# databendlabs/databend

Measured on AMD Instinct MI355X. Metric: rows/s TPC-H Q1 hash-agg, higher is better.
Workload: dtype i64/i128 decimal

## Files before the change

### databend_amd/csrc/k_parquet_dev.hip

```cpp
#include "pq_common.h"

#include <stdlib.h>
#include "dv_wave.h"

namespace {

enum { DV_OK = 0, DV_CORRUPT = 1, DV_UNSUPPORTED = 2 };
enum { ENC_DELTA_BINARY_PACKED = 5, ENC_DELTA_LENGTH_BYTE_ARRAY = 6, ENC_DELTA_BYTE_ARRAY = 7, ENC_BYTE_STREAM_SPLIT = 9 };
__host__ __device__ __forceinline__ bool dv_ext_enc(uint32_t e) {
  return e == ENC_DELTA_LENGTH_BYTE_ARRAY || e == ENC_DELTA_BYTE_ARRAY || e == ENC_BYTE_STREAM_SPLIT;
}
enum { CODEC_NONE = 0, CODEC_SNAPPY = 1, CODEC_ZSTD = 6, CODEC_LZ4_RAW = 7 };
enum { PQ_NODE_LIST = 1, PQ_NODE_STRUCT = 2 };
inline uint32_t bit_width_u32(uint32_t v) { uint32_t b = 0; for (; v; v >>= 1) ++b; return b; }

__device__ __forceinline__ void dv_fail(uint32_t* ctl, uint32_t code) { atomicCAS(&ctl[0], 0u, code); }

__device__ __forceinline__ uint32_t uni(uint32_t v) { return (uint32_t)__builtin_amdgcn_readfirstlane((int)v); }

__global__ __launch_bounds__(128) void dv_inflate_zstd2_kernel(const DvJob* __restrict__ jobs, uint32_t ring) {
  extern __shared__ __align__(16) uint8_t dv_lds[];
  const DvJob P = jobs[blockIdx.x];
  const uint32_t lane = threadIdx.x & 63, wave = threadIdx.x >> 6;
  const uint32_t lev = P.lev_len;
  const uint32_t raw = P.compressed ? lev : P.uncomp_len;
  for (uint32_t i = threadIdx.x; i < raw; i += 128) P.dst[i] = P.src[i];
  if (!P.compressed || P.uncomp_len == lev) return;
  ZQueue Q;
  Q.slots = (u32x4q*)(dv_lds + ring + ZW_TABLES);
  Q.ctl = (uint32_t*)(dv_lds + ring + ZW_TABLES + ZQ_CAP * 16);
  if (threadIdx.x < 4) Q.ctl[threadIdx.x] = 0;
  __syncthreads();
  if (wave == 0) {
    ZProd a;
    a.begin(P, dv_lds, ring, lane);
    a.qbegin(Q);
    int rc = zc::decode_frames(a, a.in_len);
    if (rc == zc::OK && a.op_ != a.cap_) rc = zc::CORRUPT_;
    a.end((uint32_t)rc);
  } else {
    ZWave b;
    b.begin(P, dv_lds, ring, lane);
    const int rc = (int)zq_consume(b, Q);
    b.flush(true);
    if (rc) dv_fail(P.ctl, rc == zc::UNSUPPORTED ? DV_UNSUPPORTED : DV_CORRUPT);
  }
}

__global__ __launch_bounds__(64) void dv_inflate_lz_kernel(const DvJob* __restrict__ jobs, uint32_t ring) {
  extern __shared__ __align__(16) uint8_t dv_lds[];
  const DvJob P = jobs[blockIdx.x];
  const uint32_t lane = threadIdx.x;
  const uint32_t lev = P.lev_len;
  const uint32_t raw = P.compressed ? lev : P.uncomp_len;
  for (uint32_t i = lane; i < raw; i += 64) P.dst[i] = P.src[i];
  if (!P.compressed || P.uncomp_len == lev) return;
  ZWave w;
  w.begin(P, dv_lds, ring, lane);
  FwdStream in;
  in.open(w.srcA, w.safeA, w.a0, lane);
  bool ok = P.codec == CODEC_SNAPPY ? snappy_raw(w, in) : lz4_block(w, in);
  if (ok && w.op_ != w.cap_) ok = false;
  w.flush(true);
  if (!ok) dv_fail(P.ctl, DV_CORRUPT);
}

__device__ __forceinline__ uint64_t dv_peek8(const uint8_t* __restrict__ s, uint32_t pos, uint32_t len) {
  uint64_t v = 0;
#pragma unroll
  for (int k = 0; k < 8; ++k)
    if (pos + (uint32_t)k < len) v |= (uint64_t)s[pos + k] << (8 * k);
  return v;
}

__device__ __forceinline__ bool dv_varint(const uint8_t* __restrict__ s, uint32_t* pos, uint32_t len, uint64_t* out) {
  const uint64_t w = dv_peek8(s, *pos, len);
  uint64_t v = 0;
  for (int k = 0; k < 8; ++k) {
    if (*pos + (uint32_t)k >= len) return false;
    const uint32_t b = (uint32_t)(w >> (8 * k)) & 0xFFu;
    v |= (uint64_t)(b & 0x7F) << (7 * k);
    if (!(b & 0x80)) { *pos += (uint32_t)k + 1; *out = v; return true; }
  }
  for (int k = 8; k < 10; ++k) {
    if (*pos + (uint32_t)k >= len) return false;
    const uint32_t b = s[*pos + k];
    v |= (uint64_t)(b & 0x7F) << (7 * k);
    if (!(b & 0x80)) { *pos += (uint32_t)k + 1; *out = v; return true; }
  }
  return false;
}

template <class Rle, class Bp>
__device__ __forceinline__ bool dv_walk_hybrid(const uint8_t* __restrict__ s, uint32_t len, int bitw, uint32_t nvals, Rle&& rle, Bp&& bp) {
// ... 490 lines not shown
  } else if (cv.esize == 16) {
    ((i128*)out)[o] = (i128)(int64_t)v;
  } else {
    ((uint64_t*)out)[o] = v;
  }
}

__device__ __forceinline__ uint64_t dv_unpack64(const uint8_t* __restrict__ src, uint32_t i, uint32_t b) {
  if (b == 0) return 0;
  const uint64_t bit = (uint64_t)i * b;
  const uint8_t* p = src + (bit >> 3);
  const uint32_t sh = (uint32_t)(bit & 7);
  const uint32_t nb = (sh + b + 7) >> 3;
  uint64_t v = load_le(p, nb < 8 ? (int)nb : 8) >> sh;
  if (nb > 8) v |= (uint64_t)p[8] << (64 - sh);
  return b >= 64 ? v : (v & ((1ull << b) - 1));
}

struct DvDeltaShared {
  uint64_t wt[4];
};

template <class Put>
__device__ __forceinline__ bool dv_delta_walk(const uint8_t* __restrict__ s, uint32_t rlen, uint32_t count, bool exact, DvDeltaShared* S, Put&& put,
                                              uint32_t* end) {
  const uint32_t tid = threadIdx.x;
  uint32_t pos = 0;
  uint64_t bs, mb, total, zz;
  if (!dv_varint(s, &pos, rlen, &bs) || !dv_varint(s, &pos, rlen, &mb) || !dv_varint(s, &pos, rlen, &total) || !dv_varint(s, &pos, rlen, &zz))
    return false;
  if (mb == 0 || mb > 4096 || bs == 0 || bs > (1u << 24) || bs % mb != 0) return false;
  const uint32_t vpm = (uint32_t)(bs / mb);
  if (vpm % 8 != 0) return false;
  if (total < (uint64_t)count || (exact && total != (uint64_t)count)) return false;
  *end = pos;
  if (count == 0) return true;
  uint64_t last = (zz >> 1) ^ (0 - (zz & 1));
  if (tid == 0) put(0u, last);
  uint32_t produced = 1;
  while (produced < count) {
    uint64_t mz;
    if (!dv_varint(s, &pos, rlen, &mz)) return false;
    const uint64_t min_delta = (mz >> 1) ^ (0 - (mz & 1));
    if (rlen - pos < (uint32_t)mb) return false;
    const uint32_t bwpos = pos;
    pos += (uint32_t)mb;
    for (uint32_t m = 0; m < (uint32_t)mb && produced < count; ++m) {
      const uint32_t b = s[bwpos + m];
      if (b > 64) return false;
      const uint32_t need = (count - produced) < vpm ? (count - produced) : vpm;
      const uint64_t need_bytes = ((uint64_t)need * b + 7) >> 3;
      if ((uint64_t)(rlen - pos) < need_bytes) return false;
      for (uint32_t c0 = 0; c0 < need; c0 += 256) {
        const uint32_t i = c0 + tid;
        const uint64_t dlt = i < need ? min_delta + dv_unpack64(s + pos, i, b) : 0;
        uint64_t incl = dlt;
        for (int dd = 1; dd < 64; dd <<= 1) {
          const uint64_t t = __shfl_up(incl, dd, 64);
          if ((int)(tid & 63) >= dd) incl += t;
        }
        __syncthreads();
        if ((tid & 63) == 63) S->wt[tid >> 6] = incl;
        __syncthreads();
        uint64_t wb = last;
        for (uint32_t w = 0; w < (tid >> 6); ++w) wb += S->wt[w];
        if (i < need) put(produced + i, wb + incl);
        last += S->wt[0] + S->wt[1] + S->wt[2] + S->wt[3];
      }
      const uint64_t mbytes = ((uint64_t)vpm * b) >> 3;
      pos += mbytes < (uint64_t)(rlen - pos) ? (uint32_t)mbytes : rlen - pos;
      produced += need;
    }
  }
  *end = pos;
  return true;
}

__device__ bool dv_delta(const uint8_t* __restrict__ s, uint32_t rlen, uint32_t count, const PqConv& cv, void* __restrict__ out, uint64_t o0,
                         DvDeltaShared* S) {
  uint32_t end;
  return dv_delta_walk(s, rlen, count, false, S, [&](uint32_t i, uint64_t v) { dv_store_int(cv, out, o0 + i, v); }, &end);
}

__device__ __forceinline__ void dv_put_dict(const PqConv& cv, const void* __restrict__ dict, uint32_t idx, void* __restrict__ out, uint64_t o) {
  switch (cv.esize) {
    case 1: ((uint8_t*)out)[o] = ((const uint8_t*)dict)[idx]; break;
    case 2: ((uint16_t*)out)[o] = ((const uint16_t*)dict)[idx]; break;
    case 4: ((uint32_t*)out)[o] = ((const uint32_t*)dict)[idx]; break;
    case 8: ((uint64_t*)out)[o] = ((const uint64_t*)dict)[idx]; break;
    default: ((uint4*)out)[o] = ((const uint4*)dict)[idx]; break;
  }
}

union DvValShared {
  DvStrShared str;
  DvDeltaShared delta;
};

__global__ __launch_bounds__(256) void dv_dict_kernel(const DvChunkD* __restrict__ cds, const uint32_t* __restrict__ list) {
  __shared__ DvStrShared S;
  const DvChunkD& C = cds[list[blockIdx.x]];
  const uint8_t* __restrict__ img = C.img;
  const PqConv cv = C.cv;
  void* __restrict__ dict = C.dict_out;
  uint32_t* __restrict__ ctl = C.hdr;
  const DvPage P = C.pages[C.dict_page];
  if (P.num_values == 0) return;
  if (cv.physical == PT_BYTE_ARRAY) {
    if (!dv_walk_strings(img, P.img_off, P.uncomp_len, P.num_values, dict, 0, &S)) dv_fail(ctl, DV_CORRUPT);
    return;
  }
  const uint32_t w = (uint32_t)plain_width(cv.physical, cv.type_length);
  if (w == 0 || P.uncomp_len / w < P.num_values) { dv_fail(ctl, DV_CORRUPT); return; }
  for (uint32_t i = threadIdx.x; i < P.num_values; i += 256) store_plain(cv, img + P.img_off + (uint64_t)i * w, dict, i);
}

__global__ __launch_bounds__(256) void dv_values_kernel(const DvChunkD* __restrict__ cds, const uint2* __restrict__ map) {
  __shared__ DvValShared S;
  const uint2 m = map[blockIdx.x];
  const DvChunkD& C = cds[m.x];
  if (blockIdx.y >= C.slices) return;
  const uint32_t d = m.y, tid = threadIdx.x;
  const uint8_t* __restrict__ img = C.img;
  const PqConv cv = C.cv;
  const void* __restrict__ dict = C.dict;
  const uint32_t dict_n = C.dict_n;
  void* __restrict__ out = C.target;
  const uint64_t out_cap = C.rows;
  uint32_t* __restrict__ ctl = C.hdr;
  const DvPage P = C.pages[C.dp[d]];
  const uint32_t n = C.nn[d], vo = C.voff[d];
  const uint64_t o0 = C.vbase[d];
  if (n == 0) return;
  if (vo > P.uncomp_len || n > P.num_values || o0 + n > out_cap) { dv_fail(ctl, DV_CORRUPT); return; }
  const uint8_t* s = img + P.img_off + vo;
  const uint32_t rlen = P.uncomp_len - vo;
  const uint32_t enc = P.enc;
  if (enc == ENC_PLAIN && cv.physical != PT_BOOLEAN && cv.physical != PT_BYTE_ARRAY) {
    const uint32_t w = (uint32_t)plain_width(cv.physical, cv.type_length);
    if (w == 0 || rlen / w < n) { dv_fail(ctl, DV_CORRUPT); return; }
    const uint32_t lo = (uint32_t)((uint64_t)n * blockIdx.y / C.slices), hi = (uint32_t)((uint64_t)n * (blockIdx.y + 1) / C.slices);
    for (uint32_t i = lo + tid; i < hi; i += 256) store_plain(cv, s + (uint64_t)i * w, out, o0 + i);
    return;
  }
  if (blockIdx.y != 0) return;
  bool ok = true;
  if (enc == ENC_PLAIN && cv.physical == PT_BOOLEAN) {
    if ((uint64_t)rlen * 8 < n) { dv_fail(ctl, DV_CORRUPT); return; }
    (void)dv_put_bits((uint32_t*)out, o0, n, s, tid, 256);
  } else if (enc == ENC_PLAIN) {
    ok = dv_walk_strings(img, P.img_off + vo, rlen, n, out, o0, &S.str);
  } else if (enc == ENC_PLAIN_DICT || enc == ENC_RLE_DICT) {
    if (rlen < 1 || dict_n == 0 || !dict) { dv_fail(ctl, DV_CORRUPT); return; }
    const int bitw = s[0];
    if (bitw > 32) { dv_fail(ctl, DV_CORRUPT); return; }
    ok = dv_walk_hybrid(
        s + 1, rlen - 1, bitw, n,
        [&](uint32_t first, uint32_t cnt, uint32_t v) {
          if (v >= dict_n) dv_fail(ctl, DV_CORRUPT);
          const uint32_t idx = v < dict_n ? v : dict_n - 1;
          for (uint32_t i = tid; i < cnt; i += 256) dv_put_dict(cv, dict, idx, out, o0 + first + i);
        },
        [&](uint32_t first, uint32_t cnt, const uint8_t* src) {
          for (uint32_t i = tid; i < cnt; i += 256) {
            uint32_t idx = extract_bits(src, i, bitw);
            if (idx >= dict_n) { dv_fail(ctl, DV_CORRUPT); idx = dict_n - 1; }
            dv_put_dict(cv, dict, idx, out, o0 + first + i);
          }
        });
  } else if (enc == ENC_RLE && cv.physical == PT_BOOLEAN) {
    if (rlen < 4) { dv_fail(ctl, DV_CORRUPT); return; }
    const uint32_t len = (uint32_t)load_le(s, 4);
    if (len > rlen - 4) { dv_fail(ctl, DV_CORRUPT); return; }
    ok = dv_walk_hybrid(
        s + 4, len, 1, n,
        [&](uint32_t first, uint32_t cnt, uint32_t v) { if (v == 1) (void)dv_put_bits((uint32_t*)out, o0 + first, cnt, nullptr, tid, 256); },
        [&](uint32_t first, uint32_t cnt, const uint8_t* src) { (void)dv_put_bits((uint32_t*)out, o0 + first, cnt, src, tid, 256); });
  } else if (enc == ENC_DELTA_BINARY_PACKED && (cv.physical == PT_INT32 || cv.physical == PT_INT64)) {
    ok = dv_delta(s, rlen, n, cv, out, o0, &S.delta);
  } else {
    dv_fail(ctl, DV_UNSUPPORTED);
    return;
  }
  if (!ok) dv_fail(ctl, DV_CORRUPT);
}

struct DvXJob {
  uint32_t k, d;
  uint32_t enc, sec;
  uint32_t* lens;
  uint8_t* dst;
  uint64_t aoff;
  uint64_t bytes;
  uint32_t live, pad;
};

__device__ __forceinline__ void dv_view(const uint8_t* __restrict__ p, uint32_t len, uint32_t buf, uint32_t off, void* __restrict__ out, uint64_t o) {
  uint32_t w[4];
  sv_make(p, len, buf, off, w);
  ((uint4*)out)[o] = make_uint4(w[0], w[1], w[2], w[3]);
}

__device__ __forceinline__ uint64_t dv_block_xscan(uint64_t v, uint64_t* wt, uint64_t* tot) {
  const uint32_t tid = threadIdx.x;
  uint64_t incl = v;
  for (int dd = 1; dd < 64; dd <<= 1) {
    const uint64_t t = __shfl_up(incl, dd, 64);
    if ((int)(tid & 63) >= dd) incl += t;
  }
  __syncthreads();
  if ((tid & 63) == 63) wt[tid >> 6] = incl;
  __syncthreads();
  uint64_t wb = 0;
  for (uint32_t w = 0; w < (tid >> 6); ++w) wb += wt[w];
  *tot = wt[0] + wt[1] + wt[2] + wt[3];
  return wb + incl - v;
}

__device__ __forceinline__ void dv_store_bss(const PqConv& cv, const uint8_t* __restrict__ s, uint32_t n, uint32_t i, void* __restrict__ out, uint64_t o) {
  if (cv.physical == PT_FLBA) {
    const int L = cv.type_length;
    u128 v = (s[i] & 0x80) ? ~(u128)0 : (u128)0;
#pragma unroll
    for (int b = 0; b < 16; ++b)
      if (b < L) v = (v << 8) | s[(uint64_t)b * n + i];
    if (cv.esize == 16) ((u128*)out)[o] = v; else ((uint64_t*)out)[o] = (uint64_t)v;
    return;
  }
  const int w = (cv.physical == PT_INT32 || cv.physical == PT_FLOAT) ? 4 : 8;
  uint64_t v = 0;
#pragma unroll
  for (int b = 0; b < 8; ++b)
    if (b < w) v |= (uint64_t)s[(uint64_t)b * n + i] << (8 * b);
  if (w == 4) {
    const uint32_t x = (uint32_t)v;
    switch (cv.esize) {
      case 1: ((uint8_t*)out)[o] = (uint8_t)x; break;
      case 2: ((uint16_t*)out)[o] = (uint16_t)x; break;
      case 4: ((uint32_t*)out)[o] = x; break;
      default: ((int64_t*)out)[o] = (int64_t)(int32_t)x; break;
    }
    return;
  }
  if (cv.esize == 16) ((i128*)out)[o] = (i128)(int64_t)v; else ((uint64_t*)out)[o] = v;
}

__global__ __launch_bounds__(256) void dv_dba_size_kernel(const DvChunkD* __restrict__ cds, DvXJob* __restrict__ jobs) {
  __shared__ DvDeltaShared S;
  __shared__ uint64_t wt[4];
  DvXJob* J = jobs + blockIdx.x;
  const DvChunkD& C = cds[J->k];
  const uint32_t d = J->d, tid = threadIdx.x;
  uint32_t* __restrict__ ctl = C.hdr;
  const DvPage P = C.pages[C.dp[d]];
  const uint32_t n = C.nn[d], vo = C.voff[d];
  const uint64_t o0 = C.vbase[d];
  if (n == 0) return;
  if (vo > P.uncomp_len || n > P.num_values || o0 + n > C.rows) { dv_fail(ctl, DV_CORRUPT); return; }
  const uint8_t* s = C.img + P.img_off + vo;
  const uint32_t rlen = P.uncomp_len - vo;
  uint32_t* __restrict__ pre = J->lens;
  uint32_t* __restrict__ suf = J->lens + n;
  bool bad = false;
  uint32_t e1 = 0, e2 = 0;
  bool ok = dv_delta_walk(s, rlen, n, true, &S, [&](uint32_t i, uint64_t v) { bad |= (int32_t)v < 0; pre[i] = (uint32_t)v; }, &e1);
// ... 260 lines not shown
  c->image_len = codec == CODEC_NONE ? 0 : (int64_t)img + 16;
  c->known_no_nulls = c->max_def == 0 || all_v2_no_nulls;
  if (c->known_no_nulls) { c->nulls = 0; c->nonnull = c->rows; }
  if (info_host) {
    info_host->num_values = c->rows;
    info_host->num_nulls = c->known_no_nulls ? 0 : -1;
    info_host->out_type = out_type;
    info_host->has_validity = c->max_def;
    info_host->out_bytes = out_type == DBHIP_T_BOOL ? ceil_div(c->rows, 64) * 8 : c->rows * (int64_t)out_elem_size(out_type);
    info_host->validity_bytes = ceil_div(c->rows, 64) * 8;
    info_host->n_pages = c->n_pages;
    info_host->n_dict_values = c->dict_n < 0 ? 0 : c->dict_n;
    info_host->image_bytes = c->image_len;
  }
  *out_host = c;
  return DBHIP_OK;
}
}

extern "C" {

int32_t dbhip_pq_chunk_open_device(const uint8_t* chunk_host, int64_t chunk_len, int32_t codec, int32_t physical_type, int32_t type_length,
                                   int32_t max_def_level, int32_t max_rep_level, int32_t out_type, dbhip_pq_chunk** out_host,
                                   dbhip_pq_info* info_host) {
  return open_device_impl(chunk_host, chunk_len, codec, physical_type, type_length, max_def_level, max_rep_level, out_type, false, 0, 0, out_host, info_host);
}

int32_t dbhip_pq_chunk_open_device_list(const uint8_t* chunk_host, int64_t chunk_len, int32_t codec, int32_t physical_type, int32_t type_length,
                                        int32_t list_nullable, int32_t element_nullable, int32_t out_type, dbhip_pq_chunk** out_host,
                                        dbhip_pq_info* info_host) {
  DBHIP_REQUIRE((list_nullable == 0 || list_nullable == 1) && (element_nullable == 0 || element_nullable == 1), "dbhip_pq_chunk_open_device_list: nullability flags are 0 / 1");
  int32_t rc = open_device_impl(chunk_host, chunk_len, codec, physical_type, type_length, list_nullable + 1 + element_nullable, 1, out_type, true, list_nullable,
                                element_nullable, out_host, info_host);
  if (rc == DBHIP_OK && info_host) info_host->has_validity = element_nullable;
  return rc;
}

int32_t dbhip_pq_chunk_open_device_nested(const uint8_t* chunk_host, int64_t chunk_len, int32_t codec, int32_t physical_type, int32_t type_length,
                                          const dbhip_pq_node* path, int32_t n_nodes, int32_t leaf_nullable, int32_t out_type, dbhip_pq_chunk** out_host,
                                          dbhip_pq_info* info_host) {
  DBHIP_REQUIRE(out_host, "dbhip_pq_chunk_open_device_nested: NULL argument");
  *out_host = nullptr;
  DBHIP_REQUIRE(path, "dbhip_pq_chunk_open_device_nested: NULL path");
  DBHIP_REQUIRE(leaf_nullable == 0 || leaf_nullable == 1, "dbhip_pq_chunk_open_device_nested: leaf_nullable is 0 / 1");
  if (n_nodes < 1 || n_nodes > 8) {
    set_error("dbhip_pq_chunk_open_device_nested: %d path nodes (1 .. 8 are decoded)", n_nodes);
    return DBHIP_ERR_UNSUPPORTED;
  }
  int32_t lists = 0, max_def = leaf_nullable;
  for (int32_t j = 0; j < n_nodes; ++j) {
    DBHIP_REQUIRE(path[j].kind == PQ_NODE_LIST || path[j].kind == PQ_NODE_STRUCT, "dbhip_pq_chunk_open_device_nested: a node kind is LIST (1) or STRUCT (2)");
    DBHIP_REQUIRE(path[j].nullable == 0 || path[j].nullable == 1, "dbhip_pq_chunk_open_device_nested: node nullability is 0 / 1");
    lists += path[j].kind == PQ_NODE_LIST;
    max_def += path[j].nullable + (path[j].kind == PQ_NODE_LIST);
  }
  if (lists > 4) {
    set_error("dbhip_pq_chunk_open_device_nested: %d LIST nodes (at most 4 repeated levels are decoded)", lists);
    return DBHIP_ERR_UNSUPPORTED;
  }
  const int32_t rc = open_device_impl(chunk_host, chunk_len, codec, physical_type, type_length, max_def, lists, out_type, false, 0, 0, out_host, info_host, lists);
  if (rc != DBHIP_OK) return rc;
  dbhip_pq_chunk* c = *out_host;
  c->n_nodes = n_nodes; c->leaf_nullable = leaf_nullable;
  for (int32_t j = 0; j < n_nodes; ++j) { c->node_kind[j] = path[j].kind; c->node_null[j] = path[j].nullable; }
  if (info_host) info_host->has_validity = leaf_nullable;
  return DBHIP_OK;
}

}

namespace {

struct BlobLayout {
  size_t hdr, cds, dict_list, lv_map, val_map, jobs, xjobs, per_chunk, total;
};
inline size_t up16(size_t x) { return (x + 15) & ~(size_t)15; }

int32_t decode_many(dbhip_pq_chunk* const* cs, int32_t n, const uint8_t* const* chunk_dev, uint8_t* const* image_dev, void* const* out_values_dev,
                    uint8_t* const* out_validity_dev, int64_t* out_nulls_host, int32_t* out_status_host, void* stream, bool list_pass = false) {
  const char* who = "dbhip_pq_chunks_decode_device";
  if (n <= 0) return DBHIP_OK;
  hipStream_t s = resolve_stream(stream);
  size_t n_jobs = 0, n_lv = 0, n_dp = 0, per_chunk = 0;
  size_t n_ext = 0, n_dba = 0, lens_words = 0;
  std::vector<int> live;
  for (int i = 0; i < n; ++i) {
    dbhip_pq_chunk* c = cs[i];
    if (out_nulls_host) out_nulls_host[i] = 0;
    if (out_status_host) out_status_host[i] = DBHIP_OK;
    DBHIP_REQUIRE(c && c->device_mode, "dbhip_pq_chunk_decode_device: the handle was not opened by dbhip_pq_chunk_open_device");
    DBHIP_REQUIRE(!c->list || list_pass, "dbhip_pq_chunk_decode_device: a List chunk is decoded by dbhip_pq_chunk_decode_device_list");
    DBHIP_REQUIRE(!c->nested || list_pass, "dbhip_pq_chunk_decode_device: a nested leaf is decoded by dbhip_pq_chunk_decode_device_nested");
    if (c->d_arena) { (void)dbhip_free(c->d_arena); c->d_arena = nullptr; c->arena_bytes = 0; }
    if (c->rows == 0) continue;
    n_ext += (size_t)c->n_ext; n_dba += (size_t)c->n_dba; lens_words += (size_t)c->ext_lens;
    DBHIP_REQUIRE(chunk_dev[i] && out_values_dev[i], "dbhip_pq_chunk_decode_device: NULL buffer");
    DBHIP_REQUIRE(((uintptr_t)chunk_dev[i] & 15) == 0, "dbhip_pq_chunk_decode_device: chunk_dev must be 16-byte aligned");
    DBHIP_REQUIRE(c->codec == CODEC_NONE || image_dev[i], "dbhip_pq_chunk_decode_device: a compressed chunk needs an image buffer (info.image_bytes)");
    DBHIP_REQUIRE(c->codec == CODEC_NONE || ((uintptr_t)image_dev[i] & 15) == 0, "dbhip_pq_chunk_decode_device: the image buffer must be 16-byte aligned");
    DBHIP_REQUIRE(c->max_def == 0 || out_validity_dev[i], "dbhip_pq_chunk_decode_device: a nullable column needs a validity buffer");
    live.push_back(i);
    const size_t nd = c->data_pages.size();
    if (c->codec != CODEC_NONE) n_jobs += c->pages.size();
    if (c->max_def == 1) n_lv += nd;
    n_dp += nd;
    per_chunk += up16(c->pages.size() * sizeof(DvPage)) + 3 * up16(nd * 4) + up16((nd + 1) * 8);
    const int esize = out_elem_size(c->out_type);
    const bool is_bool = c->out_type == DBHIP_T_BOOL;
    const bool spread = c->max_def == 1 && !c->known_no_nulls;
    const int64_t nwords = ceil_div(c->rows, 32);
    if (c->dict_n > 0 && !c->d_dict) DBHIP_TRY(dbhip_alloc((size_t)c->dict_n * (size_t)esize, &c->d_dict));
    if (spread) {
      if (!c->d_dense) DBHIP_TRY(dbhip_alloc(is_bool ? (size_t)ceil_div(c->rows + 1, 64) * 8 : (size_t)(c->rows + 1) * (size_t)esize, &c->d_dense));
      if (!c->d_wcnt) DBHIP_TRY(dbhip_alloc((size_t)nwords * 4, (void**)&c->d_wcnt));
      if (!c->d_woff) DBHIP_TRY(dbhip_alloc((size_t)nwords * 8, (void**)&c->d_woff));
      if (!c->d_blk) DBHIP_TRY(dbhip_alloc((size_t)(ceil_div(nwords, SCAN_TILE) + 2) * 8, (void**)&c->d_blk));
    }
  }
  if (live.empty()) return DBHIP_OK;
  static const bool lds_ok = [] {
    return hipFuncSetAttribute((const void*)dv_inflate_lz_kernel, hipFuncAttributeMaxDynamicSharedMemorySize, (int)LZ_RING) == hipSuccess &&
           hipFuncSetAttribute((const void*)dv_inflate_zstd2_kernel, hipFuncAttributeMaxDynamicSharedMemorySize, (int)ZW2_LDS) == hipSuccess &&
           hipFuncSetAttribute((const void*)dv_dba_replay_kernel, hipFuncAttributeMaxDynamicSharedMemorySize, (int)LZ_RING) == hipSuccess;
  }();
  if (!lds_ok) { set_error("%s: cannot reserve LDS for the decompression kernels", who); return DBHIP_ERR_HIP; }
  const size_t nl = live.size();
  BlobLayout L;
  L.hdr = 0;
  L.cds = up16(nl * 32);
  L.dict_list = L.cds + up16(nl * sizeof(DvChunkD));
  L.lv_map = L.dict_list + up16(nl * 4);
  L.val_map = L.lv_map + up16(n_lv * 8);
  L.jobs = L.val_map + up16(n_dp * 8);
  L.xjobs = L.jobs + up16(n_jobs * sizeof(DvJob));
  L.per_chunk = L.xjobs + up16(n_ext * sizeof(DvXJob));
  L.total = L.per_chunk + per_chunk;
  uint8_t* blob = (uint8_t*)scratch(L.total, 20, s);
  if (!blob) { set_error("%s: out of device memory (%zu bytes of page tables)", who, L.total); return DBHIP_ERR_HIP; }
  uint32_t* lens = nullptr;
  if (lens_words) {
    lens = (uint32_t*)scratch(lens_words * 4 + 64, 21, s);
    if (!lens) { set_error("%s: out of device memory (%zu bytes of string lengths)", who, lens_words * 4); return DBHIP_ERR_HIP; }
  }
  std::vector<uint8_t> H(L.total, 0);
  DvChunkD* cds = (DvChunkD*)(H.data() + L.cds);
  uint32_t* dict_list = (uint32_t*)(H.data() + L.dict_list);
  uint2* lv_map = (uint2*)(H.data() + L.lv_map);
  uint2* val_map = (uint2*)(H.data() + L.val_map);
  DvJob* jobs = (DvJob*)(H.data() + L.jobs);
  DvXJob* xjobs = (DvXJob*)(H.data() + L.xjobs);
  size_t at = L.per_chunk, n_dict = 0, k_lv = 0, k_dp = 0, k_dba = 0, k_x = n_dba, lens_at = 0;
  unsigned max_slices_x = 1;
  size_t n_z = 0;
  for (int i : live)
    if (cs[i]->codec == CODEC_ZSTD) n_z += cs[i]->pages.size();
  size_t jz = 0, jo = n_z;
  bool any_list = false, any_nested = false;
  unsigned max_slices = 1;
  for (size_t k = 0; k < nl; ++k) {
    const int i = live[k];
    dbhip_pq_chunk* c = cs[i];
    const uint32_t nd = (uint32_t)c->data_pages.size();
    const int esize = out_elem_size(c->out_type);
    const bool spread = c->max_def == 1 && !c->known_no_nulls;
    DvChunkD& D = cds[k];
    auto place = [&](const void* src, size_t bytes) {
      const size_t o = at;
      if (src && bytes) memcpy(H.data() + o, src, bytes);
      at += up16(bytes);
      return blob + o;
    };
    D.pages = (const DvPage*)place(c->pages.data(), c->pages.size() * sizeof(DvPage));
    D.dp = (const uint32_t*)place(c->data_pages.data(), (size_t)nd * 4);
    D.nn = (uint32_t*)place(c->nn_init.data(), (size_t)nd * 4);
    D.voff = (uint32_t*)place(c->voff_init.data(), (size_t)nd * 4);
    D.vbase = (uint64_t*)place(nullptr, (size_t)(nd + 1) * 8);
    D.img = c->codec == CODEC_NONE ? chunk_dev[i] : image_dev[i];
    D.dict = c->d_dict; D.dict_out = c->d_dict;
    D.target = spread ? c->d_dense : out_values_dev[i];
    D.bitmap = (uint32_t*)out_validity_dev[i];
    D.hdr = (uint32_t*)(blob + L.hdr + k * 32);
    D.cv = PqConv{c->physical, c->type_length, c->out_type, esize};
    D.dict_n = (uint32_t)(c->dict_n > 0 ? c->dict_n : 0);
    D.dict_page = (uint32_t)(c->dict_page >= 0 ? c->dict_page : 0);
    D.nd = nd;
    D.rows = (uint64_t)c->rows;
    unsigned slices = 1;
    const bool fixed = c->physical != PT_BOOLEAN && c->physical != PT_BYTE_ARRAY;
    if (fixed && nd > 0) {
      const int64_t per_page = c->rows / (int64_t)nd;
      while (slices < 64 && (int64_t)n_dp * slices < 2048 && per_page / (int64_t)slices > 4096) slices <<= 1;
    }
    D.slices = slices;
    if (slices > max_slices) max_slices = slices;
    if (c->list) {
      any_list = true;
      D.ldw = c->list_max_def > 1 ? 2u : 1u; D.lmax = (uint32_t)c->list_max_def; D.lnull = (uint32_t)c->list_nullable;
      D.isrep = c->d_isrep; D.iselem = c->d_iselem; D.lvalid = c->d_lvalid;
      D.rw = 1; D.rmax = 1;
    } else if (c->nested) {
      any_list = true; any_nested = true;
      D.ldw = bit_width_u32((uint32_t)c->nest_max_def); D.lmax = (uint32_t)c->nest_max_def;
      D.rw = bit_width_u32((uint32_t)c->n_lists); D.rmax = (uint32_t)c->n_lists;
      D.lrep = c->d_lrep; D.ldef = c->d_ldef;
    }
    if (c->dict_n > 0) dict_list[n_dict++] = (uint32_t)k;
    for (uint32_t d = 0; d < nd; ++d) {
      if (c->max_def == 1) lv_map[k_lv++] = make_uint2((unsigned)k, d);
      if (c->n_ext == 0 || !dv_ext_enc(c->pages[c->data_pages[d]].enc)) { val_map[k_dp++] = make_uint2((unsigned)k, d); continue; }
      const DvPage& P = c->pages[c->data_pages[d]];
      DvXJob& X = P.enc == ENC_DELTA_BYTE_ARRAY ? xjobs[k_dba++] : xjobs[k_x++];
      X.k = (uint32_t)k; X.d = d; X.enc = P.enc;
      if (P.enc != ENC_BYTE_STREAM_SPLIT) {
        X.lens = lens + lens_at;
        lens_at += (P.enc == ENC_DELTA_BYTE_ARRAY ? 2 : 1) * (size_t)P.num_values;
      }
      if (slices > max_slices_x) max_slices_x = slices;
    }
    if (c->codec != CODEC_NONE) {
      const uint64_t safe_end = ((uint64_t)c->chunk_len + 15) & ~15ull;
      for (const DvPage& P : c->pages) {
        DvJob& J = c->codec == CODEC_ZSTD ? jobs[jz++] : jobs[jo++];
        J.src = chunk_dev[i] + P.src_off;
        J.dst = image_dev[i] + P.img_off;
        J.comp_len = P.comp_len; J.uncomp_len = P.uncomp_len; J.lev_len = P.lev_len; J.compressed = P.compressed;
        J.src_safe = (uint32_t)(safe_end - P.src_off);
        J.codec = (uint32_t)c->codec;
        J.ctl = D.hdr;
      }
    }
  }
  auto by_size = [](const DvJob& a, const DvJob& b) { return a.uncomp_len > b.uncomp_len; };
  std::sort(jobs, jobs + n_z, by_size);
  std::sort(jobs + n_z, jobs + n_jobs, by_size);
  DBHIP_CHECK(hipMemcpyAsync(blob, H.data(), L.total, hipMemcpyHostToDevice, s));
  const DvChunkD* d_cds = (const DvChunkD*)(blob + L.cds);
  const DvJob* d_jobs = (const DvJob*)(blob + L.jobs);
  for (int i : live) {
    dbhip_pq_chunk* c = cs[i];
    const bool spread = c->max_def == 1 && !c->known_no_nulls;
    uint32_t* vbits = (uint32_t*)out_validity_dev[i];
    if (c->max_def == 1) DBHIP_CHECK(hipMemsetAsync(vbits, 0, (size_t)ceil_div(c->rows, 64) * 8, s));
    else if (vbits) DBHIP_CHECK(hipMemsetAsync(vbits, 0xFF, (size_t)ceil_div(c->rows, 64) * 8, s));
    if (c->out_type == DBHIP_T_BOOL)
      DBHIP_CHECK(hipMemsetAsync(spread ? c->d_dense : out_values_dev[i], 0, (size_t)ceil_div(spread ? c->rows + 1 : c->rows, 64) * 8, s));
  }
  kernel_timer_start(s);
  if (n_z) hipLaunchKernelGGL(dv_inflate_zstd2_kernel, dim3((unsigned)n_z), dim3(128), ZW2_LDS, s, d_jobs, ZW_RING);
  if (n_jobs > n_z) hipLaunchKernelGGL(dv_inflate_lz_kernel, dim3((unsigned)(n_jobs - n_z)), dim3(64), LZ_RING, s, d_jobs + n_z, LZ_RING);
  if (n_dict) hipLaunchKernelGGL(dv_dict_kernel, dim3((unsigned)n_dict), dim3(256), 0, s, d_cds, (const uint32_t*)(blob + L.dict_list));
  if (n_lv && any_nested)
    hipLaunchKernelGGL(dv_levels_kernel<true>, dim3((unsigned)n_lv), dim3(256), LV_LDS, s, d_cds, (const uint2*)(blob + L.lv_map), LV_LDS);
  else if (n_lv)
    hipLaunchKernelGGL(dv_levels_kernel<false>, dim3((unsigned)n_lv), dim3(256), any_list ? LV_LDS : 0u, s, d_cds, (const uint2*)(blob + L.lv_map), any_list ? LV_LDS : 0u);
  hipLaunchKernelGGL(dv_scan_kernel, dim3((unsigned)nl), dim3(256), 0, s, d_cds);
  if (k_dp) hipLaunchKernelGGL(dv_values_kernel, dim3((unsigned)k_dp, max_slices), dim3(256), 0, s, d_cds, (const uint2*)(blob + L.val_map));
  DvXJob* d_xjobs = (DvXJob*)(blob + L.xjobs);
  std::vector<uint8_t> arena_unsupported(nl, 0);
  if (n_dba) {
    hipLaunchKernelGGL(dv_dba_size_kernel, dim3((unsigned)n_dba), dim3(256), 0, s, d_cds, d_xjobs);
    DBHIP_LAUNCH_CHECK();
    std::vector<uint32_t> hdr0(nl * 8, 0);
    DBHIP_CHECK(hipMemcpyAsync(hdr0.data(), blob + L.hdr, nl * 32, hipMemcpyDeviceToHost, s));
    DBHIP_CHECK(hipMemcpyAsync(xjobs, d_xjobs, n_dba * sizeof(DvXJob), hipMemcpyDeviceToHost, s));
    DBHIP_CHECK(hipStreamSynchronize(s));
    std::vector<uint64_t> total(nl, 0);
    for (size_t j = 0; j < n_dba; ++j) {
      const uint32_t k = xjobs[j].k;
      if (xjobs[j].bytes >= (1ull << 31)) arena_unsupported[k] = 1;
      xjobs[j].aoff = total[k];
      total[k] += xjobs[j].bytes;
    }
    for (size_t k = 0; k < nl; ++k) {
      if (total[k] >= (1ull << 32)) arena_unsupported[k] = 1;
      if (total[k] == 0 || hdr0[k * 8] != DV_OK || arena_unsupported[k]) continue;
      dbhip_pq_chunk* c = cs[live[k]];
      DBHIP_TRY(dbhip_alloc((size_t)total[k] + 16, &c->d_arena));
      c->arena_bytes = (int64_t)total[k];
    }
    for (size_t j = 0; j < n_dba; ++j) {
      const uint32_t k = xjobs[j].k;
      dbhip_pq_chunk* c = cs[live[k]];
      xjobs[j].live = hdr0[k * 8] == DV_OK && !arena_unsupported[k];
      xjobs[j].dst = c->d_arena ? (uint8_t*)c->d_arena + xjobs[j].aoff : nullptr;
    }
    DBHIP_CHECK(hipMemcpyAsync(d_xjobs, xjobs, n_dba * sizeof(DvXJob), hipMemcpyHostToDevice, s));
    hipLaunchKernelGGL(dv_dba_replay_kernel, dim3((unsigned)n_dba), dim3(64), LZ_RING, s, d_cds, (const DvXJob*)d_xjobs, LZ_RING);
  }
  if (n_ext) hipLaunchKernelGGL(dv_values_ext_kernel, dim3((unsigned)n_ext, max_slices_x), dim3(256), 0, s, d_cds, (const DvXJob*)d_xjobs);
  for (int i : live) {
    dbhip_pq_chunk* c = cs[i];
    if (!(c->max_def == 1 && !c->known_no_nulls)) continue;
    const int esize = out_elem_size(c->out_type);
    const int64_t nwords = ceil_div(c->rows, 32);
    uint32_t* vbits = (uint32_t*)out_validity_dev[i];
    void* out = out_values_dev[i];
    hipLaunchKernelGGL(pq_popc_kernel, dim3(grid_for(nwords, 256)), dim3(256), 0, s, vbits, nwords, c->d_wcnt);
    DBHIP_TRY(dbscan::exclusive_scan_u32(c->d_wcnt, nwords, c->d_blk, c->d_woff, s));
    const int grid = grid_for(c->rows, 256);
    if (c->out_type == DBHIP_T_BOOL) {
      hipLaunchKernelGGL(pq_spread_bool_kernel, dim3(grid_for(nwords, 256)), dim3(256), 0, s, vbits, c->d_woff, (const uint32_t*)c->d_dense, nwords, (uint32_t*)out);
      if (nwords & 1) DBHIP_CHECK(hipMemsetAsync((uint32_t*)out + nwords, 0, 4, s));
    } else if (esize == 1) {
      hipLaunchKernelGGL(pq_spread_kernel<uint8_t>, dim3(grid), dim3(256), 0, s, vbits, c->d_woff, (const uint8_t*)c->d_dense, c->rows, (uint8_t*)out);
    } else if (esize == 2) {
      hipLaunchKernelGGL(pq_spread_kernel<uint16_t>, dim3(grid), dim3(256), 0, s, vbits, c->d_woff, (const uint16_t*)c->d_dense, c->rows, (uint16_t*)out);
    } else if (esize == 4) {
      hipLaunchKernelGGL(pq_spread_kernel<uint32_t>, dim3(grid), dim3(256), 0, s, vbits, c->d_woff, (const uint32_t*)c->d_dense, c->rows, (uint32_t*)out);
    } else if (esize == 8) {
      hipLaunchKernelGGL(pq_spread_kernel<uint64_t>, dim3(grid), dim3(256), 0, s, vbits, c->d_woff, (const uint64_t*)c->d_dense, c->rows, (uint64_t*)out);
    } else {
      hipLaunchKernelGGL(pq_spread_kernel<uint4>, dim3(grid), dim3(256), 0, s, vbits, c->d_woff, (const uint4*)c->d_dense, c->rows, (uint4*)out);
    }
  }
  kernel_timer_stop(s);
  DBHIP_LAUNCH_CHECK();
  std::vector<uint32_t> hdr(nl * 8, 0);
  DBHIP_CHECK(hipMemcpyAsync(hdr.data(), blob + L.hdr, nl * 32, hipMemcpyDeviceToHost, s));
  DBHIP_CHECK(hipStreamSynchronize(s));
  int32_t first_rc = DBHIP_OK;
  for (size_t k = 0; k < nl; ++k) {
    const int i = live[k];
    dbhip_pq_chunk* c = cs[i];
    const uint32_t verdict = hdr[k * 8];
    uint64_t nonnull;
    memcpy(&nonnull, &hdr[k * 8 + 2], 8);
    int32_t rc = DBHIP_OK;
    if (verdict == DV_OK && arena_unsupported[k]) {
      set_error("dbhip_pq_chunk_decode_device: chunk %d: its DELTA_BYTE_ARRAY values take 4 GiB or more (or 2 GiB or more in one page); "
                "use the CPU reader for this chunk", i);
      rc = DBHIP_ERR_UNSUPPORTED;
    } else if (verdict == DV_UNSUPPORTED) {
      set_error("dbhip_pq_chunk_decode_device: chunk %d uses a form the device path does not decode (a Snappy back-reference beyond 64 KiB, a ZSTD "
                "dictionary, or an encoding that changes between pages); use dbhip_pq_chunk_open", i);
      rc = DBHIP_ERR_UNSUPPORTED;
    } else if (verdict != DV_OK) {
      set_error("dbhip_pq_chunk_decode_device: malformed column chunk %d (a page does not decompress to its declared size, or a level / index / "
                "length stream runs past its page)", i);
      rc = DBHIP_ERR_INVALID;
// ... 410 lines not shown
```

Baseline: 94.01 billion.

## Add dedicated dictionary-decode kernel with LDS-staged pages and LDS dictionary

Moves dictionary-encoded data pages out of the generic values kernel into a new kernel. It stages the RLE/bit-packed index stream into an LDS tile, keeps small dictionaries (element size at least 4 bytes, up to 16KB) resident in LDS, and emits outputs as 16-byte vector stores with lane rotation across runs. The goal is to cut repeated global byte reads during hybrid walking and scattered dictionary gathers. The cost is a larger dynamic LDS footprint per block, which may lower occupancy, plus an extra kernel launch.

```diff
diff --git a/databend_amd/csrc/k_parquet_dev.hip b/databend_amd/csrc/k_parquet_dev.hip
--- a/databend_amd/csrc/k_parquet_dev.hip
+++ b/databend_amd/csrc/k_parquet_dev.hip
@@ -2,6 +2,7 @@
 
 #include <stdlib.h>
 #include "dv_wave.h"
+#include "pq_hybrid.h"
 
 namespace {
 
@@ -10,6 +11,7 @@
 __host__ __device__ __forceinline__ bool dv_ext_enc(uint32_t e) {
   return e == ENC_DELTA_LENGTH_BYTE_ARRAY || e == ENC_DELTA_BYTE_ARRAY || e == ENC_BYTE_STREAM_SPLIT;
 }
+inline bool dv_dict_enc(uint32_t e) { return e == ENC_PLAIN_DICT || e == ENC_RLE_DICT; }
 enum { CODEC_NONE = 0, CODEC_SNAPPY = 1, CODEC_ZSTD = 6, CODEC_LZ4_RAW = 7 };
 enum { PQ_NODE_LIST = 1, PQ_NODE_STRUCT = 2 };
 inline uint32_t bit_width_u32(uint32_t v) { uint32_t b = 0; for (; v; v >>= 1) ++b; return b; }
@@ -666,16 +668,6 @@
   return dv_delta_walk(s, rlen, count, false, S, [&](uint32_t i, uint64_t v) { dv_store_int(cv, out, o0 + i, v); }, &end);
 }
 
-__device__ __forceinline__ void dv_put_dict(const PqConv& cv, const void* __restrict__ dict, uint32_t idx, void* __restrict__ out, uint64_t o) {
-  switch (cv.esize) {
-    case 1: ((uint8_t*)out)[o] = ((const uint8_t*)dict)[idx]; break;
-    case 2: ((uint16_t*)out)[o] = ((const uint16_t*)dict)[idx]; break;
-    case 4: ((uint32_t*)out)[o] = ((const uint32_t*)dict)[idx]; break;
-    case 8: ((uint64_t*)out)[o] = ((const uint64_t*)dict)[idx]; break;
-    default: ((uint4*)out)[o] = ((const uint4*)dict)[idx]; break;
-  }
-}
-
 union DvValShared {
   DvStrShared str;
   DvDeltaShared delta;
@@ -707,8 +699,6 @@
   const uint32_t d = m.y, tid = threadIdx.x;
   const uint8_t* __restrict__ img = C.img;
   const PqConv cv = C.cv;
-  const void* __restrict__ dict = C.dict;
-  const uint32_t dict_n = C.dict_n;
   void* __restrict__ out = C.target;
   const uint64_t out_cap = C.rows;
   uint32_t* __restrict__ ctl = C.hdr;
@@ -734,24 +724,6 @@
     (void)dv_put_bits((uint32_t*)out, o0, n, s, tid, 256);
   } else if (enc == ENC_PLAIN) {
     ok = dv_walk_strings(img, P.img_off + vo, rlen, n, out, o0, &S.str);
-  } else if (enc == ENC_PLAIN_DICT || enc == ENC_RLE_DICT) {
-    if (rlen < 1 || dict_n == 0 || !dict) { dv_fail(ctl, DV_CORRUPT); return; }
-    const int bitw = s[0];
-    if (bitw > 32) { dv_fail(ctl, DV_CORRUPT); return; }
-    ok = dv_walk_hybrid(
-        s + 1, rlen - 1, bitw, n,
-        [&](uint32_t first, uint32_t cnt, uint32_t v) {
-          if (v >= dict_n) dv_fail(ctl, DV_CORRUPT);
-          const uint32_t idx = v < dict_n ? v : dict_n - 1;
-          for (uint32_t i = tid; i < cnt; i += 256) dv_put_dict(cv, dict, idx, out, o0 + first + i);
-        },
-        [&](uint32_t first, uint32_t cnt, const uint8_t* src) {
-          for (uint32_t i = tid; i < cnt; i += 256) {
-            uint32_t idx = extract_bits(src, i, bitw);
-            if (idx >= dict_n) { dv_fail(ctl, DV_CORRUPT); idx = dict_n - 1; }
-            dv_put_dict(cv, dict, idx, out, o0 + first + i);
-          }
-        });
   } else if (enc == ENC_RLE && cv.physical == PT_BOOLEAN) {
     if (rlen < 4) { dv_fail(ctl, DV_CORRUPT); return; }
     const uint32_t len = (uint32_t)load_le(s, 4);
@@ -765,6 +737,146 @@
   } else {
     dv_fail(ctl, DV_UNSUPPORTED);
     return;
+  }
+  if (!ok) dv_fail(ctl, DV_CORRUPT);
+}
+
+#ifndef DD_TILE_BYTES
+#define DD_TILE_BYTES 16384
+#endif
+constexpr uint32_t DD_TILE = DD_TILE_BYTES;
+constexpr uint32_t DD_PAD = 32;
+constexpr uint32_t DD_DICT_BUDGET = 16384;
+
+template <int E> struct DdVal;
+template <> struct DdVal<1> { typedef uint8_t T; };
+template <> struct DdVal<2> { typedef uint16_t T; };
+template <> struct DdVal<4> { typedef uint32_t T; };
+template <> struct DdVal<8> { typedef uint64_t T; };
+template <> struct DdVal<16> { typedef u32x4q T; };
+#define DD_GLOBAL __attribute__((address_space(1)))
+
+template <class T>
+__device__ __forceinline__ T dd_lds_get(uint32_t a) { return *(const __attribute__((address_space(3))) T*)(uintptr_t)a; }
+
+template <int E, bool DL>
+struct DdWalk {
+  typedef typename DdVal<E>::T T;
+  static constexpr uint32_t V = E >= 4 ? 16 / E : 1;
+  uint32_t lo, hi, x0;
+  uint32_t tile, cap;
+  const uint8_t* s;
+  uint32_t len;
+  uint32_t dl;
+  const void* dict;
+  uint32_t dict_n;
+  void* out;
+  uint64_t o0;
+  uint32_t* ctl;
+  int bitw;
+  uint32_t tid, rot;
+
+  __device__ __forceinline__ uint32_t uni(uint32_t v) const { return (uint32_t)__builtin_amdgcn_readfirstlane((int)v); }
+  __device__ __forceinline__ uint32_t dword(uint32_t k) const { return *(const __attribute__((address_space(3))) uint32_t*)(uintptr_t)(tile + 4 * k); }
+  __device__ __forceinline__ void stage(uint32_t pos) {
+    const uint8_t* p0 = s + pos;
+    const uint32_t a = (uint32_t)((uintptr_t)p0 & 15u);
+    const uint8_t* pa = p0 - a;
+    const uint32_t n = len - pos < cap ? len - pos : cap, have = n + a;
+    __syncthreads();
+    for (uint32_t x = tid * 16; x < have; x += 4 * 256 * 16) {
+      u32x4q r[4];
+#pragma unroll
+      for (uint32_t j = 0; j < 4; ++j)
+        if (x + j * 4096 < have) r[j] = *(const DD_GLOBAL u32x4q*)(pa + x + j * 4096);
+#pragma unroll
+      for (uint32_t j = 0; j < 4; ++j)
+        if (x + j * 4096 < have) *(__attribute__((address_space(3))) u32x4q*)(uintptr_t)(tile + x + j * 4096) = r[j];
+    }
+    __syncthreads();
+    lo = uni(pos); hi = uni(pos + n); x0 = uni(a);
+  }
+  __device__ __forceinline__ T lookup(uint32_t idx) const {
+    if (idx >= dict_n) { dv_fail(ctl, DV_CORRUPT); idx = dict_n - 1; }
+    if (DL) return dd_lds_get<T>(dl + idx * (uint32_t)E);
+    return ((const DD_GLOBAL T*)dict)[idx];
+  }
+  template <class Val>
+  __device__ __forceinline__ void emit(uint32_t first, uint32_t n, Val&& val) {
+    DD_GLOBAL T* o = (DD_GLOBAL T*)((T*)out + (o0 + first));
+    if (V == 1) {
+      for (uint32_t i = (tid - rot) & 255u; i < n; i += 256) o[i] = val(i);
+      rot = (rot + n) & 255u;
+      return;
+    }
+    uint32_t h = ((0u - (uint32_t)(uintptr_t)o) & 15u) / (uint32_t)E;
+    if (h > n) h = n;
+    const uint32_t nch = (n - h) / V, t0 = h + nch * V;
+    if (tid < h) o[tid] = val(tid);
+    else if (tid - h < n - t0) o[t0 + tid - h] = val(t0 + tid - h);
+    for (uint32_t c = (tid - rot) & 255u; c < nch; c += 256) {
+      const uint32_t i = h + c * V;
+      union { T v[V]; u32x4q q; } pk;
+#pragma unroll
+      for (uint32_t j = 0; j < V; ++j) pk.v[j] = val(i + j);
+      *(DD_GLOBAL u32x4q*)(o + i) = pk.q;
+    }
+    rot = (rot + nch) & 255u;
+  }
+  __device__ __forceinline__ void rle(uint32_t first, uint32_t n, uint32_t v) {
+    const T x = lookup(v);
+    emit(first, n, [&](uint32_t) { return x; });
+  }
+  __device__ __forceinline__ void bp(uint32_t first, uint32_t n, uint32_t pos) {
+    emit(first, n, [&](uint32_t i) { return lookup(hy::index_at(*this, pos, i, bitw)); });
+  }
+};
+
+template <int E, bool DL>
+__device__ __forceinline__ bool dd_run(uint32_t tile, uint32_t cap, uint32_t dl, const uint8_t* s, uint32_t len, int bitw, uint32_t n, const void* dict,
+                                       uint32_t dict_n, void* out, uint64_t o0, uint32_t* ctl) {
+  DdWalk<E, DL> W;
+  W.lo = 0; W.hi = 0; W.x0 = 0;
+  W.tile = tile; W.cap = cap; W.s = s; W.len = len; W.dl = dl; W.dict = dict; W.dict_n = dict_n; W.out = out; W.o0 = o0; W.ctl = ctl;
+  W.bitw = bitw; W.tid = threadIdx.x; W.rot = 0;
+  return hy::walk(W, len, bitw, n);
+}
+
+__global__ __launch_bounds__(256) void dv_values_dict_kernel(const DvChunkD* __restrict__ cds, const uint2* __restrict__ map, uint32_t cap, uint32_t dict_cap) {
+  extern __shared__ __align__(16) uint8_t dd_lds[];
+  const uint2 m = map[blockIdx.x];
+  const DvChunkD& C = cds[m.x];
+  const uint32_t d = m.y, tid = threadIdx.x;
+  const PqConv cv = C.cv;
+  const void* __restrict__ dict = C.dict;
+  const uint32_t dict_n = C.dict_n;
+  void* __restrict__ out = C.target;
+  uint32_t* __restrict__ ctl = C.hdr;
+  const DvPage P = C.pages[C.dp[d]];
+  const uint32_t n = C.nn[d], vo = C.voff[d];
+  const uint64_t o0 = C.vbase[d];
+  if (n == 0) return;
+  if (vo > P.uncomp_len || n > P.num_values || o0 + n > C.rows) { dv_fail(ctl, DV_CORRUPT); return; }
+  const uint8_t* s = C.img + P.img_off + vo;
+  const uint32_t rlen = P.uncomp_len - vo;
+  if (rlen < 1 || dict_n == 0 || !dict) { dv_fail(ctl, DV_CORRUPT); return; }
+  const int bitw = *(const DD_GLOBAL uint8_t*)s;
+  if (bitw > 32) { dv_fail(ctl, DV_CORRUPT); return; }
+  const uint32_t tile = (uint32_t)(uintptr_t)dd_lds, dl = tile + cap + DD_PAD;
+  const uint32_t esize = (uint32_t)cv.esize;
+  const bool in_lds = esize >= 4 && (uint64_t)dict_n * esize <= (uint64_t)dict_cap;
+  if (in_lds)
+    for (uint32_t x = tid; x < dict_n * (esize / 4); x += 256) *(__attribute__((address_space(3))) uint32_t*)(uintptr_t)(dl + 4 * x) = ((const DD_GLOBAL uint32_t*)dict)[x];
+  bool ok;
+  switch (esize) {
+    case 1: ok = dd_run<1, false>(tile, cap, dl, s + 1, rlen - 1, bitw, n, dict, dict_n, out, o0, ctl); break;
+    case 2: ok = dd_run<2, false>(tile, cap, dl, s + 1, rlen - 1, bitw, n, dict, dict_n, out, o0, ctl); break;
+    case 4: ok = in_lds ? dd_run<4, true>(tile, cap, dl, s + 1, rlen - 1, bitw, n, dict, dict_n, out, o0, ctl)
+                        : dd_run<4, false>(tile, cap, dl, s + 1, rlen - 1, bitw, n, dict, dict_n, out, o0, ctl); break;
+    case 8: ok = in_lds ? dd_run<8, true>(tile, cap, dl, s + 1, rlen - 1, bitw, n, dict, dict_n, out, o0, ctl)
+                        : dd_run<8, false>(tile, cap, dl, s + 1, rlen - 1, bitw, n, dict, dict_n, out, o0, ctl); break;
+    default: ok = in_lds ? dd_run<16, true>(tile, cap, dl, s + 1, rlen - 1, bitw, n, dict, dict_n, out, o0, ctl)
+                         : dd_run<16, false>(tile, cap, dl, s + 1, rlen - 1, bitw, n, dict, dict_n, out, o0, ctl); break;
   }
   if (!ok) dv_fail(ctl, DV_CORRUPT);
 }
@@ -1191,6 +1303,7 @@
   if (n <= 0) return DBHIP_OK;
   hipStream_t s = resolve_stream(stream);
   size_t n_jobs = 0, n_lv = 0, n_dp = 0, per_chunk = 0;
+  size_t n_dd = 0, dd_dict = 0;
   size_t n_ext = 0, n_dba = 0, lens_words = 0;
   std::vector<int> live;
   for (int i = 0; i < n; ++i) {
@@ -1215,6 +1328,11 @@
     n_dp += nd;
     per_chunk += up16(c->pages.size() * sizeof(DvPage)) + 3 * up16(nd * 4) + up16((nd + 1) * 8);
     const int esize = out_elem_size(c->out_type);
+    for (uint32_t dp : c->data_pages) n_dd += dv_dict_enc(c->pages[dp].enc);
+    if (c->dict_n > 0) {
+      const uint64_t db = (uint64_t)c->dict_n * (uint64_t)esize;
+      if (esize >= 4 && db <= DD_DICT_BUDGET && db > dd_dict) dd_dict = (size_t)db;
+    }
     const bool is_bool = c->out_type == DBHIP_T_BOOL;
     const bool spread = c->max_def == 1 && !c->known_no_nulls;
     const int64_t nwords = ceil_div(c->rows, 32);
@@ -1230,7 +1348,8 @@
   static const bool lds_ok = [] {
     return hipFuncSetAttribute((const void*)dv_inflate_lz_kernel, hipFuncAttributeMaxDynamicSharedMemorySize, (int)LZ_RING) == hipSuccess &&
            hipFuncSetAttribute((const void*)dv_inflate_zstd2_kernel, hipFuncAttributeMaxDynamicSharedMemorySize, (int)ZW2_LDS) == hipSuccess &&
-           hipFuncSetAttribute((const void*)dv_dba_replay_kernel, hipFuncAttributeMaxDynamicSharedMemorySize, (int)LZ_RING) == hipSuccess;
+           hipFuncSetAttribute((const void*)dv_dba_replay_kernel, hipFuncAttributeMaxDynamicSharedMemorySize, (int)LZ_RING) == hipSuccess &&
+           hipFuncSetAttribute((const void*)dv_values_dict_kernel, hipFuncAttributeMaxDynamicSharedMemorySize, (int)(DD_TILE + DD_PAD + DD_DICT_BUDGET)) == hipSuccess;
   }();
   if (!lds_ok) { set_error("%s: cannot reserve LDS for the decompression kernels", who); return DBHIP_ERR_HIP; }
   const size_t nl = live.size();
@@ -1258,7 +1377,8 @@
   uint2* val_map = (uint2*)(H.data() + L.val_map);
   DvJob* jobs = (DvJob*)(H.data() + L.jobs);
   DvXJob* xjobs = (DvXJob*)(H.data() + L.xjobs);
-  size_t at = L.per_chunk, n_dict = 0, k_lv = 0, k_dp = 0, k_dba = 0, k_x = n_dba, lens_at = 0;
+  const size_t dd_at = n_dp - n_dd;
+  size_t at = L.per_chunk, n_dict = 0, k_lv = 0, k_dp = 0, k_dd = 0, k_dba = 0, k_x = n_dba, lens_at = 0;
   unsigned max_slices_x = 1;
   size_t n_z = 0;
   for (int i : live)
@@ -1316,6 +1436,7 @@
     if (c->dict_n > 0) dict_list[n_dict++] = (uint32_t)k;
     for (uint32_t d = 0; d < nd; ++d) {
       if (c->max_def == 1) lv_map[k_lv++] = make_uint2((unsigned)k, d);
+      if (dv_dict_enc(c->pages[c->data_pages[d]].enc)) { val_map[dd_at + k_dd++] = make_uint2((unsigned)k, d); continue; }
       if (c->n_ext == 0 || !dv_ext_enc(c->pages[c->data_pages[d]].enc)) { val_map[k_dp++] = make_uint2((unsigned)k, d); continue; }
       const DvPage& P = c->pages[c->data_pages[d]];
       DvXJob& X = P.enc == ENC_DELTA_BYTE_ARRAY ? xjobs[k_dba++] : xjobs[k_x++];
@@ -1364,6 +1485,11 @@
     hipLaunchKernelGGL(dv_levels_kernel<false>, dim3((unsigned)n_lv), dim3(256), any_list ? LV_LDS : 0u, s, d_cds, (const uint2*)(blob + L.lv_map), any_list ? LV_LDS : 0u);
   hipLaunchKernelGGL(dv_scan_kernel, dim3((unsigned)nl), dim3(256), 0, s, d_cds);
   if (k_dp) hipLaunchKernelGGL(dv_values_kernel, dim3((unsigned)k_dp, max_slices), dim3(256), 0, s, d_cds, (const uint2*)(blob + L.val_map));
+  if (k_dd) {
+    const uint32_t cap = DD_TILE, dict_cap = (uint32_t)up16(dd_dict);
+    hipLaunchKernelGGL(dv_values_dict_kernel, dim3((unsigned)k_dd), dim3(256), cap + DD_PAD + dict_cap, s, d_cds, (const uint2*)(blob + L.val_map) + dd_at, cap,
+                       dict_cap);
+  }
   DvXJob* d_xjobs = (DvXJob*)(blob + L.xjobs);
   std::vector<uint8_t> arena_unsupported(nl, 0);
   if (n_dba) {
diff --git a/databend_amd/csrc/pq_hybrid.h b/databend_amd/csrc/pq_hybrid.h
--- /dev/null
+++ b/databend_amd/csrc/pq_hybrid.h
@@ -0,0 +1,121 @@
+#pragma once
+#include <stdint.h>
+
+#if defined(__HIPCC__)
+#define HY_FN __device__ __forceinline__
+#else
+#define HY_FN static inline
+#endif
+
+namespace hy {
+
+enum { HDR_SPAN = 14 };
+enum { MIN_TILE = 64 };
+enum { MAX_BITW = 32 };
+
+template <class B>
+HY_FN uint64_t peek8(B& b, uint32_t pos) {
+  const uint32_t a = pos - b.lo + b.x0, k = a >> 2, sft = 8 * (a & 3);
+  const uint32_t d0 = b.dword(k), d1 = b.dword(k + 1), d2 = b.dword(k + 2);
+  const uint64_t w = (uint64_t)d0 | ((uint64_t)d1 << 32);
+  const uint64_t r = sft ? (w >> sft) | ((uint64_t)d2 << (64 - sft)) : w;
+  return (uint64_t)b.uni((uint32_t)r) | ((uint64_t)b.uni((uint32_t)(r >> 32)) << 32);
+}
+
+template <class B>
+HY_FN uint32_t index_at(B& b, uint32_t pos, uint32_t i, int bitw) {
+  const uint32_t bit = (pos - b.lo + b.x0) * 8 + i * (uint32_t)bitw;
+  const uint32_t k = bit >> 5, sh = bit & 31;
+  const uint64_t w = (uint64_t)b.dword(k) | ((uint64_t)b.dword(k + 1) << 32);
+  return (uint32_t)(w >> sh) & (bitw >= 32 ? 0xFFFFFFFFu : ((1u << bitw) - 1));
+}
+
+template <class B>
+HY_FN bool varint(B& b, uint32_t* pos, uint32_t len, uint64_t* out) {
+  const uint32_t p = *pos;
+  if (p >= len) return false;
+  const uint32_t room = len - p;
+  const uint64_t w = peek8(b, p);
+  uint64_t v = 0;
+  for (uint32_t k = 0; k < 8; ++k) {
+    if (k >= room) return false;
+    const uint32_t c = (uint32_t)(w >> (8 * k)) & 0xFFu;
+    v |= (uint64_t)(c & 0x7F) << (7 * k);
+    if (!(c & 0x80)) { *pos = p + k + 1; *out = v; return true; }
+  }
+  if (room <= 8) return false;
+  const uint64_t w2 = peek8(b, p + 8);
+  for (uint32_t k = 8; k < 10; ++k) {
+    if (k >= room) return false;
+    const uint32_t c = (uint32_t)(w2 >> (8 * (k - 8))) & 0xFFu;
+    v |= (uint64_t)(c & 0x7F) << (7 * k);
+    if (!(c & 0x80)) { *pos = p + k + 1; *out = v; return true; }
+  }
+  return false;
+}
+
+HY_FN uint32_t values_staged(uint32_t p, uint32_t hi, int bitw, uint32_t left) {
+  const uint32_t bits = (hi - p) * 8u;
+  if ((uint64_t)left * (uint32_t)bitw <= (uint64_t)bits) return left;
+  return (bits / (uint32_t)bitw) & ~7u;
+}
+
+template <class B>
+HY_FN bool walk(B& b, uint32_t len, int bitw, uint32_t nvals) {
+  if (bitw < 0 || bitw > MAX_BITW) return false;
+  uint32_t pos = 0, done = 0;
+  const uint32_t vbytes = (uint32_t)(bitw + 7) >> 3;
+  while (done < nvals) {
+    if (pos >= len) return false;
+    if (pos < b.lo || pos >= b.hi || (b.hi < len && b.hi - pos < (uint32_t)HDR_SPAN)) b.stage(pos);
+    uint64_t h;
+    if (!varint(b, &pos, len, &h)) return false;
+    pos = b.uni(pos);
+    const uint32_t avail = len - pos;
+    if (h & 1) {
+      const uint64_t groups = h >> 1;
+      if (groups == 0 || groups > 0x1FFFFFFFull) return false;
+      const uint64_t n64 = groups * 8;
+      const uint32_t n = n64 > (uint64_t)(nvals - done) ? nvals - done : (uint32_t)n64;
+      if ((uint64_t)n * (uint64_t)bitw > (uint64_t)avail * 8) return false;
+      if (bitw == 0) {
+        b.rle(done, n, 0u);
+      } else {
+        uint32_t p = pos, first = done, left = n;
+        while (left) {
+          bool fresh = false;
+          if (p < b.lo || p >= b.hi) { b.stage(p); fresh = true; }
+          uint32_t take = values_staged(p, b.hi, bitw, left);
+          if (take == 0) {
+            if (fresh) return false;
+            b.stage(p);
+            take = values_staged(p, b.hi, bitw, left);
+            if (take == 0) return false;
+          }
+          b.bp(first, take, p);
+          first += take; left -= take;
+          p = b.uni(p + (take >> 3) * (uint32_t)bitw);
+        }
+      }
+      const uint64_t bytes = groups * (uint64_t)bitw;
+      pos = b.uni(pos + (bytes < (uint64_t)avail ? (uint32_t)bytes : avail));
+      done = b.uni(done + n);
+    } else {
+      const uint64_t n64 = h >> 1;
+      if (n64 == 0 || avail < vbytes) return false;
+      uint32_t v = 0;
+      if (vbytes) {
+        const uint64_t w = peek8(b, pos);
+        v = vbytes >= 4 ? (uint32_t)w : ((uint32_t)w & ((1u << (8 * vbytes)) - 1));
+      }
+      pos = b.uni(pos + vbytes);
+      if (bitw < 32 && (v >> bitw) != 0) return false;
+      const uint32_t n = n64 > (uint64_t)(nvals - done) ? nvals - done : (uint32_t)n64;
+      b.rle(done, n, v);
+      done = b.uni(done + n);
+    }
+  }
+  return true;
+}
+
+}
```

Result: no change. 94.06 billion (median of 3 runs) (+0.0%).
